# orottier/web-audio-api-rs

Measured on AMD Instinct MI355X. Metric: render quanta/sec (48kHz, 128-frame), higher is better.
Workload: dtype f64

## Files before the change

### web-audio-api-rs_amd/csrc/waa_biquad_stream.hip

```cpp
#include <hip/hip_runtime.h>

#include <cstdlib>

#include "waa_internal.hpp"
#include "waa_stream_common.hpp"

namespace waa {

namespace {
struct M2 {
  double a, b, c, d;
};
__device__ __forceinline__ M2 mm(const M2& x, const M2& y) {
  M2 r;
  r.a = __builtin_fma(x.a, y.a, x.b * y.c);
  r.b = __builtin_fma(x.a, y.b, x.b * y.d);
  r.c = __builtin_fma(x.c, y.a, x.d * y.c);
  r.d = __builtin_fma(x.c, y.b, x.d * y.d);
  return r;
}

}

__device__ unsigned long long g_stream_trace[8192 * 4];

template <int DBG, int VARY, int NBUF = 2, bool DUP = false>
__global__ __launch_bounds__(64, 2) void biquad_stream_kernel_t(const BiquadStreamDesc d) {
  extern __shared__ __attribute__((aligned(16))) float lds[];
  const uint32_t wid = blockIdx.x;
  const uint32_t inst = wid / (uint32_t)d.nch;
  const int ch = (int)(wid % (uint32_t)d.nch);
  const int lane = threadIdx.x;
  if (inst >= d.n_inst) return;

  __builtin_amdgcn_s_setreg(1 | (6 << 6) | (1 << 11), 0);
  unsigned long long trace_t0 = 0;
  if constexpr (DBG == 7) trace_t0 = wall_clock64();

  const double* cp = d.coefs + (uint64_t)inst * d.coef_stride;
  double b0 = cp[0], b1 = cp[1], b2 = cp[2], a1 = cp[3], a2 = cp[4];
  M2 A1;
  {
    M2 m = {-a1, -a2, 1., 0.};
#pragma unroll
    for (int s = 0; s < 5; s++) m = mm(m, m);
    A1 = m;
  }
  const M2 A2 = mm(A1, A1), A4 = mm(A2, A2), A8 = mm(A4, A4), A16 = mm(A8, A8);
  M2 Aj = {1., 0., 0., 1.};
  if constexpr (VARY == 0) {
    const int j = lane & 15;
    if (j & 1) Aj = mm(Aj, A1);
    if (j & 2) Aj = mm(Aj, A2);
    if (j & 4) Aj = mm(Aj, A4);
    if (j & 8) Aj = mm(Aj, A8);
  }
  const int row = lane >> 4;

  double* st = d.state + (uint64_t)inst * STATE_STRIDE + ch * 4;
  double cx1 = st[0], cx2 = st[1], cy1 = st[2], cy2 = st[3];

  float g[2] = {1.f, 1.f};
  bool g_mute[2] = {false, false}, g_pass[2] = {true, true};
#pragma unroll
  for (int k = 0; k < 2; k++)
    if (k < d.n_gain) {
      g[k] = d.gain[k].base[inst];
      g_mute[k] = fabsf(g[k]) <= 1e-6f;
      g_pass[k] = fabsf(1.f - g[k]) <= 1e-6f;
    }

  const bool is_src = d.in.kind == IN_SOURCE;
  SrcInst si{};
  SrcSchedule sc{};
  const float* sig_base = nullptr;
  if (is_src) {
    si = d.in.src[inst];
    sc = si.sc;
  } else {
    sig_base = d.in.sig.base + (uint64_t)inst * d.in.sig.inst_stride + (uint64_t)ch * d.in.sig.ch_stride;
  }
  float* out_base = d.out.base + (uint64_t)inst * d.out.inst_stride + (uint64_t)ch * d.out.ch_stride;

  auto lds_sync = []() __attribute__((always_inline)) { __builtin_amdgcn_wave_barrier(); };

  auto fetch_fast = [&](uint32_t tile, float (&dst)[TILE_K]) __attribute__((always_inline)) {
    const float* p = is_src ? si.base + (uint64_t)ch * si.ch_stride +
                                  (tile < si.fast_prefix ? si.linear_start + (int64_t)tile * TILE
                                                         : load_global(&sc.qrec[(uint64_t)tile * QUANTA_PER_TILE].start))
                            : sig_base + (uint64_t)tile * TILE;
#pragma unroll
    for (int j = 0; j < NV4; j++) {
      const f4v t = DBG == 5 ? load_global_f4(p + j * 256 + lane * 4)
                             : __builtin_nontemporal_load((const WAA_GLOBAL_AS f4v*)(p + j * 256 + lane * 4));
      dst[j * 4 + 0] = t.x;
      dst[j * 4 + 1] = t.y;
      dst[j * 4 + 2] = t.z;
      dst[j * 4 + 3] = t.w;
    }
  };
  auto tile_is_fast = [&](uint32_t tile) __attribute__((always_inline)) -> bool {
    return !is_src || tile < si.fast_prefix || (si.aligned && load_global(sc.tile_fast + tile));
  };

  auto stage = [&](const float (&cur)[TILE_K]) __attribute__((always_inline)) {
#pragma unroll
    for (int j = 0; j < NV4; j++) {
      const int r = j * 8 + (lane >> 3), c = (lane & 7) * 4;
      *reinterpret_cast<float4*>(lds + r * LDS_ROW + c) =
          make_float4(cur[j * 4 + 0], cur[j * 4 + 1], cur[j * 4 + 2], cur[j * 4 + 3]);
    }
  };
  float* lds_out = lds + 64 * LDS_ROW;
  auto flush = [&](uint32_t tile) __attribute__((always_inline)) {
    lds_sync();
    float* op = out_base + (uint64_t)tile * TILE;
#pragma unroll
    for (int j = 0; j < NV4; j++) {
      const int r = j * 8 + (lane >> 3), c = (lane & 7) * 4;
      float4 t = *reinterpret_cast<const float4*>(lds_out + r * LDS_ROW + c);
#pragma unroll
      for (int k = 0; k < 2; k++)
        if (k < d.n_gain) {
          if (g_mute[k]) {
            t = make_float4(0.f, 0.f, 0.f, 0.f);
          } else if (!g_pass[k]) {
            t.x *= g[k];
            t.y *= g[k];
            t.z *= g[k];
            t.w *= g[k];
          }
        }
      if constexpr (DBG == 2) {
        asm volatile("" ::"v"(t.x), "v"(t.y), "v"(t.z), "v"(t.w));
      } else if constexpr (DBG == 5) {
        *reinterpret_cast<float4*>(op + j * 256 + lane * 4) = t;
      } else {
        __builtin_nontemporal_store(f4v{t.x, t.y, t.z, t.w}, (WAA_GLOBAL_AS f4v*)(op + j * 256 + lane * 4));
        if constexpr (DUP)
          __builtin_nontemporal_store(f4v{t.x, t.y, t.z, t.w}, (WAA_GLOBAL_AS f4v*)(op + d.out.ch_stride + j * 256 + lane * 4));
      }
    }
    lds_sync();
  };
  auto process_arate = [&](uint32_t tile) __attribute__((always_inline)) {
    lds_sync();
    const float* xrow = lds + lane * LDS_ROW;
    float* yrow = lds_out + lane * LDS_ROW;
    const double* ct = cp + (uint64_t)tile * (TILE_K * 5 * 64) + lane;
    auto load_chunk = [&](double (&c)[20], int chunk) __attribute__((always_inline)) {
      if (DBG >= 3 && tile != d.tile0) return;
#pragma unroll
      for (int j = 0; j < 20; j++) c[j] = load_global(ct + (chunk * 20 + j) * 64);
    };
    const float xl1 = xrow[TILE_K - 1], xl2 = xrow[TILE_K - 2];
    const float xm1 = __shfl_up(xl1, 1, 64), xm2 = __shfl_up(xl2, 1, 64);
// ... 127 lines not shown
            load_chunk(ca, chunk + 3);
            step_b(cb, chunk + 1);
            load_chunk(cb, chunk + 4);
            step_b(cc, chunk + 2);
          }
          step_b(ca, 6);
          step_b(cb, 7);
        } else {
#pragma unroll 1
          for (int chunk = 0; chunk < TILE_K / 4; chunk += 2) {
            step_b(ca, chunk);
            if (chunk + 2 < TILE_K / 4) load_chunk(ca, chunk + 2);
            step_b(cb, chunk + 1);
            if (chunk + 3 < TILE_K / 4) load_chunk(cb, chunk + 3);
          }
        }
      };
      sweep(false);
      if (__any(badacc != badacc)) {
        y1 = __builtin_isfinite(s1) ? s1 : 0.;
        y2 = __builtin_isfinite(s2) ? s2 : 0.;
        load_chunk(ca, 0);
        load_chunk(cb, 1);
        sweep(true);
      }
      cx1 = (double)__int_as_float(__builtin_amdgcn_readlane(__float_as_int(xl1), 63));
      cx2 = (double)__int_as_float(__builtin_amdgcn_readlane(__float_as_int(xl2), 63));
      cy1 = read_lane(y1, 63);
      cy2 = read_lane(y2, 63);
    }
    lds_sync();
  };
  auto process = [&](uint32_t tile) __attribute__((always_inline)) {
    lds_sync();
    float x[TILE_K];
#pragma unroll
    for (int j = 0; j < NV4; j++) {
      const float4 t = *reinterpret_cast<const float4*>(lds + lane * LDS_ROW + j * 4);
      x[j * 4 + 0] = t.x;
      x[j * 4 + 1] = t.y;
      x[j * 4 + 2] = t.z;
      x[j * 4 + 3] = t.w;
    }
    if constexpr (DBG == 1) {
      lds_sync();
#pragma unroll
      for (int j = 0; j < NV4; j++)
        *reinterpret_cast<float4*>(lds_out + lane * LDS_ROW + j * 4) =
            make_float4(x[j * 4 + 0], x[j * 4 + 1], x[j * 4 + 2], x[j * 4 + 3]);
      lds_sync();
      return;
    }
    M2 Al = A1;
    if constexpr (VARY == 1) {
      uint32_t q = tile * QUANTA_PER_TILE + (lane >> 2);
      if (q >= d.n_quanta) q = d.n_quanta - 1;
      const double* cq = cp + (uint64_t)q * 5;
      b0 = cq[0];
      b1 = cq[1];
      b2 = cq[2];
      a1 = cq[3];
      a2 = cq[4];
      M2 m = {-a1, -a2, 1., 0.};
#pragma unroll
      for (int s = 0; s < 5; s++) m = mm(m, m);
      Al = m;
    }
    const float xm1 = __shfl_up(x[TILE_K - 1], 1, 64), xm2 = __shfl_up(x[TILE_K - 2], 1, 64);
    double x1 = lane == 0 ? cx1 : (double)xm1;
    double x2 = lane == 0 ? cx2 : (double)xm2;
    double w[TILE_K];
    double z1 = 0., z2 = 0.;
#pragma unroll
    for (int i = 0; i < TILE_K; i++) {
      const double xd = (double)x[i];
      w[i] = (b0 * xd + b1 * x1) + b2 * x2;
      x2 = x1;
      x1 = xd;
      const double t = __builtin_fma(-a2, z2, w[i]);
      const double y = __builtin_fma(-a1, z1, t);
      z2 = z1;
      z1 = y;
    }
    double s1, s2;
    if constexpr (VARY == 0) {
      double r1 = z1, r2 = z2;
      {
        double q1 = row_shr<1>(r1), q2 = row_shr<1>(r2);
        r1 = __builtin_fma(A1.a, q1, __builtin_fma(A1.b, q2, r1));
        r2 = __builtin_fma(A1.c, q1, __builtin_fma(A1.d, q2, r2));
        q1 = row_shr<2>(r1);
        q2 = row_shr<2>(r2);
        r1 = __builtin_fma(A2.a, q1, __builtin_fma(A2.b, q2, r1));
        r2 = __builtin_fma(A2.c, q1, __builtin_fma(A2.d, q2, r2));
        q1 = row_shr<4>(r1);
        q2 = row_shr<4>(r2);
        r1 = __builtin_fma(A4.a, q1, __builtin_fma(A4.b, q2, r1));
        r2 = __builtin_fma(A4.c, q1, __builtin_fma(A4.d, q2, r2));
        q1 = row_shr<8>(r1);
        q2 = row_shr<8>(r2);
        r1 = __builtin_fma(A8.a, q1, __builtin_fma(A8.b, q2, r1));
        r2 = __builtin_fma(A8.c, q1, __builtin_fma(A8.d, q2, r2));
      }
      const double e01 = read_lane(r1, 15), e02 = read_lane(r2, 15);
      const double e11 = read_lane(r1, 31), e12 = read_lane(r2, 31);
      const double e21 = read_lane(r1, 47), e22 = read_lane(r2, 47);
      const double t01 = cy1, t02 = cy2;
      const double t11 = __builtin_fma(A16.a, t01, __builtin_fma(A16.b, t02, e01));
      const double t12 = __builtin_fma(A16.c, t01, __builtin_fma(A16.d, t02, e02));
      const double t21 = __builtin_fma(A16.a, t11, __builtin_fma(A16.b, t12, e11));
      const double t22 = __builtin_fma(A16.c, t11, __builtin_fma(A16.d, t12, e12));
      const double t31 = __builtin_fma(A16.a, t21, __builtin_fma(A16.b, t22, e21));
      const double t32 = __builtin_fma(A16.c, t21, __builtin_fma(A16.d, t22, e22));
      const double T1 = row == 0 ? t01 : row == 1 ? t11 : row == 2 ? t21 : t31;
      const double T2 = row == 0 ? t02 : row == 1 ? t12 : row == 2 ? t22 : t32;
      const double ex1 = row_shr<1>(r1), ex2 = row_shr<1>(r2);
      s1 = __builtin_fma(Aj.a, T1, __builtin_fma(Aj.b, T2, ex1));
      s2 = __builtin_fma(Aj.c, T1, __builtin_fma(Aj.d, T2, ex2));
    } else {
      M2 P = Al;
      double r1 = z1, r2 = z2;
      auto step = [&](auto shr) __attribute__((always_inline)) {
        M2 Q;
        Q.a = shr(P.a, 1.);
        Q.b = shr(P.b, 0.);
        Q.c = shr(P.c, 0.);
        Q.d = shr(P.d, 1.);
        const double q1 = shr(r1, 0.), q2 = shr(r2, 0.);
        r1 = __builtin_fma(P.a, q1, __builtin_fma(P.b, q2, r1));
        r2 = __builtin_fma(P.c, q1, __builtin_fma(P.d, q2, r2));
        P = mm(P, Q);
      };
      step([](double v, double idv) __attribute__((always_inline)) { return row_shr_keep<1>(v, idv); });
      step([](double v, double idv) __attribute__((always_inline)) { return row_shr_keep<2>(v, idv); });
      step([](double v, double idv) __attribute__((always_inline)) { return row_shr_keep<4>(v, idv); });
      step([](double v, double idv) __attribute__((always_inline)) { return row_shr_keep<8>(v, idv); });
      double t1[4], t2[4];
      t1[0] = cy1;
      t2[0] = cy2;
#pragma unroll
      for (int k = 0; k < 3; k++) {
        const int e = 16 * k + 15;
        const double pa = read_lane(P.a, e), pb = read_lane(P.b, e), pc = read_lane(P.c, e), pd = read_lane(P.d, e);
        const double e1 = read_lane(r1, e), e2 = read_lane(r2, e);
        t1[k + 1] = __builtin_fma(pa, t1[k], __builtin_fma(pb, t2[k], e1));
        t2[k + 1] = __builtin_fma(pc, t1[k], __builtin_fma(pd, t2[k], e2));
      }
      const double T1 = row == 0 ? t1[0] : row == 1 ? t1[1] : row == 2 ? t1[2] : t1[3];
      const double T2 = row == 0 ? t2[0] : row == 1 ? t2[1] : row == 2 ? t2[2] : t2[3];
      const double xa = row_shr_keep<1>(P.a, 1.), xb = row_shr_keep<1>(P.b, 0.), xc = row_shr_keep<1>(P.c, 0.),
                   xd = row_shr_keep<1>(P.d, 1.);
      const double x1r = row_shr_keep<1>(r1, 0.), x2r = row_shr_keep<1>(r2, 0.);
      s1 = __builtin_fma(xa, T1, __builtin_fma(xb, T2, x1r));
      s2 = __builtin_fma(xc, T1, __builtin_fma(xd, T2, x2r));
    }
    double y1 = s1, y2 = s2;
    float badacc = 0.f;
    float yo[TILE_K];
#pragma unroll
    for (int i = 0; i < TILE_K; i++) {
      const double y = (w[i] - a1 * y1) - a2 * y2;
      y2 = y1;
      y1 = y;
      yo[i] = (float)y;
      badacc = __builtin_fmaf(yo[i], 0.f, badacc);
    }
    if (__any(badacc != badacc)) {
      y1 = s1;
      y2 = s2;
      if (!__builtin_isfinite(y1)) y1 = 0.;
      if (!__builtin_isfinite(y2)) y2 = 0.;
#pragma unroll
      for (int i = 0; i < TILE_K; i++) {
        double y = (w[i] - a1 * y1) - a2 * y2;
        if (!__builtin_isnormal(y)) y = 0.;
        y2 = y1;
        y1 = y;
        yo[i] = (float)y;
      }
    }
    cx1 = (double)__int_as_float(__builtin_amdgcn_readlane(__float_as_int(x[TILE_K - 1]), 63));
    cx2 = (double)__int_as_float(__builtin_amdgcn_readlane(__float_as_int(x[TILE_K - 2]), 63));
    cy1 = read_lane(y1, 63);
    cy2 = read_lane(y2, 63);
    lds_sync();
#pragma unroll
    for (int j = 0; j < NV4; j++)
      *reinterpret_cast<float4*>(lds_out + lane * LDS_ROW + j * 4) =
          make_float4(yo[j * 4 + 0], yo[j * 4 + 1], yo[j * 4 + 2], yo[j * 4 + 3]);
    lds_sync();
  };

  bool pending = false;
  uint32_t pending_tile = 0;
  uint32_t tile = d.tile0;
  while (tile < d.tile1) {
    if (!tile_is_fast(tile)) {
      float tmp[TILE_K];
      load_channel_generic(d.in, si, sc, ch, tile, lane, d.n_quanta, tmp);
      float cur[TILE_K];
#pragma unroll
      for (int i = 0; i < TILE_K; i++) cur[i] = tmp[i];
      stage(cur);
      if (pending) flush(pending_tile);
      if constexpr (VARY >= 2) process_arate(tile); else process(tile);
      pending = true;
      pending_tile = tile;
      tile++;
      continue;
    }
    uint32_t end = tile + 1;
    if (is_src && end < si.fast_prefix) end = si.fast_prefix < d.tile1 ? si.fast_prefix : d.tile1;
    while (end < d.tile1 && tile_is_fast(end)) end++;
    if constexpr (VARY == 0 && NBUF == 4) {
      float na[TILE_K], nb[TILE_K];
      fetch_fast(tile, na);
      fetch_fast(tile + 1 < end ? tile + 1 : tile, nb);
      for (; tile + 1 < end; tile += 2) {
        stage(na);
        fetch_fast(tile + 2 < end ? tile + 2 : tile, na);
        if (pending) flush(pending_tile);
        process(tile);
        pending = true;
        pending_tile = tile;
        stage(nb);
        fetch_fast(tile + 3 < end ? tile + 3 : tile + 1, nb);
        flush(pending_tile);
        process(tile + 1);
        pending_tile = tile + 1;
      }
      if (tile < end) {
        stage(na);
        if (pending) flush(pending_tile);
        process(tile);
        pending = true;
        pending_tile = tile;
        tile++;
      }
      continue;
    }
    float nx[TILE_K];
    fetch_fast(tile, nx);
    for (; tile < end; tile++) {
      stage(nx);
      fetch_fast(tile + 1 < end ? tile + 1 : tile, nx);
      if (pending) flush(pending_tile);
      if constexpr (VARY >= 2) process_arate(tile); else process(tile);
      pending = true;
      pending_tile = tile;
    }
  }
  if (pending) flush(pending_tile);
  if (lane == 0) {
    st[0] = cx1;
    st[1] = cx2;
    st[2] = cy1;
    st[3] = cy2;
  }
  if constexpr (DBG == 7) {
    if (lane == 0 && wid < 8192) {
      g_stream_trace[wid * 4 + 0] = trace_t0;
      g_stream_trace[wid * 4 + 1] = wall_clock64();
      g_stream_trace[wid * 4 + 2] = __builtin_amdgcn_s_getreg(4 | (0 << 6) | (31 << 11));
      g_stream_trace[wid * 4 + 3] = __builtin_amdgcn_s_getreg(20 | (0 << 6) | (31 << 11));
    }
  }
}

__global__ __launch_bounds__(64, 4) void biquad_stream_digest_kernel(const BiquadStreamDesc d) {
  extern __shared__ __attribute__((aligned(16))) float lds[];
  double* htab = reinterpret_cast<double*>(lds + 64 * LDS_ROW);
  const uint32_t wid = blockIdx.x;
  const uint32_t inst = wid / (uint32_t)d.nch;
  const int ch = (int)(wid % (uint32_t)d.nch);
  const int lane = threadIdx.x;
  if (inst >= d.n_inst) return;
  __builtin_amdgcn_s_setreg(1 | (6 << 6) | (1 << 11), 0);

  auto uni = [](double v) __attribute__((always_inline)) {
    return __hiloint2double(__builtin_amdgcn_readfirstlane(__double2hiint(v)), __builtin_amdgcn_readfirstlane(__double2loint(v)));
  };
  auto uni_m = [&](const M2& m) __attribute__((always_inline)) { return M2{uni(m.a), uni(m.b), uni(m.c), uni(m.d)}; };
  const double* cp = d.coefs + (uint64_t)inst * d.coef_stride;
  const double b0 = uni(cp[0]), b1 = uni(cp[1]), b2 = uni(cp[2]), a1 = uni(cp[3]), a2 = uni(cp[4]);
  M2 A1;
  {
    M2 m = {-a1, -a2, 1., 0.};
#pragma unroll
    for (int s = 0; s < 5; s++) m = mm(m, m);
    A1 = uni_m(m);
  }
  const M2 A2 = uni_m(mm(A1, A1)), A4 = uni_m(mm(A2, A2)), A8 = uni_m(mm(A4, A4)), A16 = uni_m(mm(A8, A8));
  M2 Aj = {1., 0., 0., 1.};
  {
    const int j = lane & 15;
    if (j & 1) Aj = mm(Aj, A1);
    if (j & 2) Aj = mm(Aj, A2);
    if (j & 4) Aj = mm(Aj, A4);
    if (j & 8) Aj = mm(Aj, A8);
  }
// ... 238 lines not shown
    if (!tile_is_fast(tile)) {
      float tmp[TILE_K];
      load_channel_generic(d.in, si, sc, ch, tile, lane, d.n_quanta, tmp);
      float cur[TILE_K];
#pragma unroll
      for (int i = 0; i < TILE_K; i++) cur[i] = tmp[i];
      swap_in(cur, have, done);
      process();
      have = true;
      done = tile;
      tile++;
      continue;
    }
    uint32_t end = tile + 1;
    if (is_src && end < si.fast_prefix) end = si.fast_prefix < d.tile1 ? si.fast_prefix : d.tile1;
    while (end < d.tile1 && tile_is_fast(end)) end++;
    float nx[TILE_K];
    fetch_fast(tile, nx);
    for (; tile < end; tile++) {
      swap_in(nx, have, done);
      fetch_fast(tile + 1 < end ? tile + 1 : tile, nx);
      process();
      have = true;
      done = tile;
    }
  }
  if (have) flush_last(done);
  if (lane == 0) {
    st[0] = cx1;
    st[1] = cx2;
    st[2] = cy1;
    st[3] = cy2;
  }
}

void launch_biquad_stream(const BiquadStreamDesc& d, void* stream) {
  const dim3 grid(d.n_inst * (uint32_t)d.nch), block(64);
  const size_t lds = 2 * 64 * LDS_ROW * sizeof(float);
  const char* dbg = measure_switch("WAA_STREAM_DEBUG");
  if (d.dup_out && d.vary == 0) {
    hipLaunchKernelGGL((biquad_stream_kernel_t<0, 0, 4, true>), grid, block, lds, (hipStream_t)stream, d);
    return;
  }
  if (d.vary == 3 && dbg && dbg[0] == '3')
    hipLaunchKernelGGL((biquad_stream_kernel_t<3, 3>), grid, block, lds, (hipStream_t)stream, d);
  else if (d.vary == 3 && dbg && dbg[0] == '4')
    hipLaunchKernelGGL((biquad_stream_kernel_t<4, 3>), grid, block, lds, (hipStream_t)stream, d);
  else if (d.vary == 3 && measure_switch("WAA_ARATE_BUFS3"))
    hipLaunchKernelGGL((biquad_stream_kernel_t<0, 3, 3>), grid, block, lds, (hipStream_t)stream, d);
  else if (d.vary == 3)
    hipLaunchKernelGGL((biquad_stream_kernel_t<0, 3>), grid, block, lds, (hipStream_t)stream, d);
  else if (d.vary == 2)
    hipLaunchKernelGGL((biquad_stream_kernel_t<0, 2>), grid, block, lds, (hipStream_t)stream, d);
  else if (d.vary)
    hipLaunchKernelGGL((biquad_stream_kernel_t<0, 1>), grid, block, lds, (hipStream_t)stream, d);
  else if (dbg && dbg[0] == '1')
    hipLaunchKernelGGL((biquad_stream_kernel_t<1, 0>), grid, block, lds, (hipStream_t)stream, d);
  else if (dbg && dbg[0] == '2')
    hipLaunchKernelGGL((biquad_stream_kernel_t<2, 0>), grid, block, lds, (hipStream_t)stream, d);
  else if (dbg && dbg[0] == '5')
    hipLaunchKernelGGL((biquad_stream_kernel_t<5, 0>), grid, block, lds, (hipStream_t)stream, d);
  else if (dbg && dbg[0] == '7')
    hipLaunchKernelGGL((biquad_stream_kernel_t<7, 0>), grid, block, lds, (hipStream_t)stream, d);
  else if (measure_switch("WAA_STREAM_PREFETCH1"))
    hipLaunchKernelGGL((biquad_stream_kernel_t<0, 0, 2>), grid, block, lds, (hipStream_t)stream, d);
  else if (measure_switch("WAA_BIQUAD_DIGEST"))
    hipLaunchKernelGGL(biquad_stream_digest_kernel, grid, block, 64 * LDS_ROW * sizeof(float) + 34 * 2 * sizeof(double),
                       (hipStream_t)stream, d);
  else
    hipLaunchKernelGGL((biquad_stream_kernel_t<0, 0, 4>), grid, block, lds, (hipStream_t)stream, d);
}

}

extern "C" int waa_debug_stream_trace(unsigned long long* dst, unsigned n_words) {
  return (int)hipMemcpyFromSymbol(dst, HIP_SYMBOL(waa::g_stream_trace), (size_t)n_words * 8);
}
```

### web-audio-api-rs_amd/csrc/waa_internal.hpp

```cpp
#pragma once
#include <cstdint>
#include <cstdlib>

#include "waa_conv_noise.hpp"

namespace waa {

inline const char* measure_switch(const char* name) {
#ifdef WAA_MEASURE
  return getenv(name);
#else
  (void)name;
  return nullptr;
#endif
}

void raise_lds_limit(const void* kernel);

constexpr int RQ = 128;
constexpr int TILE_K = 32;
constexpr int TILE = 64 * TILE_K;
constexpr int QUANTA_PER_TILE = TILE / RQ;
constexpr int MAX_OPS = 12;
constexpr int MAX_INPUTS = 4;
// ... 78 lines not shown
  int32_t nch_out;
  int32_t i1;
  int32_t i2;
  int32_t i0;
  ParamRef p0;
  ParamRef p1;
  ParamRef p2;
  ParamRef p3;
  ParamRef p4;
  const void* ptr0;
  void* ptr1;
  const void* ptr2;
  uint64_t u0;
};

struct ChainDesc {
  int32_t n_inputs;
  int32_t in_nch;
  int32_t in_interp;
  int32_t n_ops;
  InputRef in[MAX_INPUTS];
  OpDesc ops[MAX_OPS];
  SignalRef out;
  uint32_t n_inst;
  uint32_t n_tiles;
  uint32_t n_quanta;
  uint32_t xcd_remap;
  uint32_t tile0, tile1;
  int32_t lds_curve_op;
  int32_t tile_major;
  uint32_t persist_block;
  uint32_t pad;
};

struct BiquadStreamDesc {
  InputRef in;
  const double* coefs;
  uint64_t coef_stride;
  int32_t vary;
  int32_t pad0;
  double* state;
  const double* hp;
  ParamRef gain[2];
  int32_t n_gain;
  int32_t nch;
  SignalRef out;
  uint32_t n_inst;
  uint32_t n_tiles;
  uint32_t n_quanta;
  uint32_t dup_out;
  uint32_t tile0, tile1;
};
void launch_biquad_stream(const BiquadStreamDesc& d, void* stream);
constexpr int BIQUAD_SCAN_PW = 88;
struct BiquadScanCtl {
  uint32_t* counter;
  uint32_t counter_base[8];
  double* payload;
  const double* pw;
  uint32_t* error;
};
void launch_biquad_scan_powers(const double* coefs, uint64_t coef_stride, double* pw, uint32_t n_inst, void* stream);
void launch_biquad_scan(const BiquadStreamDesc& d, const BiquadScanCtl& ctl, uint32_t* issued, void* stream);

constexpr int BIQUAD_HT_WORDS = 2 * TILE + 8;
struct BiquadLanesDesc {
  InputRef in;
  const double* coefs;
  double* ht;
  double* z;
  double* sin;
  double* state;
  ParamRef gain[2];
  int32_t n_gain, nch;
  SignalRef out;
  uint32_t n_inst, n_tiles, n_quanta, tile0, tile1;
  uint32_t fast_tiles;
  uint32_t lt0, lt1;
  uint32_t debug, pad;
};
void launch_biquad_tile_digest(const BiquadLanesDesc& d, void* stream);
void launch_biquad_lanes(const BiquadLanesDesc& d, void* stream);

struct IirStreamDesc {
  InputRef in;
  const double* coef;
  const double* pow;
  double* state;
  int32_t ns;
  int32_t nch;
  SignalRef out;
  uint32_t n_inst;
  uint32_t n_tiles;
  uint32_t n_quanta;
  uint32_t exact;
  uint32_t tile0, tile1;
};
int iir_padded_states(int n_states);
void launch_iir_stream(const IirStreamDesc& d, void* stream);

struct CompRow {
  float thr, lo, hi, half_knee;
  float knee_partial, ratio, makeup, pad;
  float a_tau, a_one, r_tau, r_one;
};
struct CompDesc {
// ... 524 lines not shown
```

### web-audio-api-rs_amd/csrc/waa_plan.cpp

```cpp
#include <array>
#include <set>

#include <memory>

#include "waa_host.hpp"
#include "waa_plan_parts.hpp"

namespace waa {
namespace host {

int prepare_source_input(waa_batch* b, uint32_t id, InputRef* in);
int validate_plan(waa_batch* b);

int device_timeline_param(waa_batch* b, const ParamStore& p, ParamRef* ref) {
  if (p.dev_ready) {
    *ref = p.dev_ref;
    return 0;
  }
  std::vector<TlHeader> hdr(b->n_inst);
  std::vector<TlEvent> events;
  std::vector<float> curves;
  for (uint32_t i = 0; i < b->n_inst; i++) {
    TlHeader& h = hdr[i];
    std::memset(&h, 0, sizeof h);
// ... 705 lines not shown
      for (size_t k = i + 1; k < j; k++) L.gain[k - i - 1] = ops[k].p0;
      L.nch = cur_nch;
      L.out = seg_out;
      L.n_inst = b->n_inst;
      L.n_tiles = b->n_tiles;
      L.n_quanta = b->n_quanta;
      L.tile0 = 0;
      L.tile1 = b->n_tiles;
      L.fast_tiles = inputs[0].kind == IN_SOURCE ? inputs[0].fast_tiles
                                                 : (inputs[0].valid ? (uint32_t)std::min<uint64_t>(inputs[0].valid / TILE, b->n_tiles) : b->n_tiles);
      dstep.kind = 18;
      dstep.lanes = L;
      dstep.profile_slot = slot_for(b, "biquad_tile_digest_kernel");
      Step ls;
      ls.kind = 19;
      ls.lanes = L;
      ls.profile_slot = slot_for(b, "biquad_lanes_kernel");
      b->steps.push_back(ls);
      plan_note(b, "biquad_lanes(a-rate, shared table: one lane per stream, tiles in parallel) in=%s:%dch gains=%d out=%s",
                input_kind_name(inputs[0].kind), cur_nch, L.n_gain, seg_out.base == out.base ? "final" : "temp");
      InputRef in{};
      in.kind = IN_SIGNAL;
      in.nch = cur_nch;
      in.sig = seg_out;
      inputs.assign(1, in);
      in_nch = cur_nch;
      i = j;
      if (i == ops.size() && seg_out.base == out.base) return 0;
      continue;
    }
    Step st;
    st.kind = 1;
    BiquadStreamDesc& q = st.bq;
    std::memset(&q, 0, sizeof q);
    q.in = inputs[0];
    q.coefs = reinterpret_cast<const double*>(o.ptr0);
    q.coef_stride = o.u0;
    q.vary = o.i0;
    if (o.i0 == 2) {
      Step& cstep = b->steps[(size_t)o.i1];
      cstep.coef.lane_major = 1;
      if (cstep.coef.rows == 1 && !measure_switch("WAA_NO_ARATE_DIGEST")) {
        Step& hstep = b->steps[(size_t)o.i1 + 1];
        double* dhp = nullptr;
        int e = dev_alloc(b, &dhp, (size_t)b->n_tiles * HP_WORDS * 64);
        if (e) return e;
        hstep.hp.coefs = cstep.coef.coefs;
        hstep.hp.hp = dhp;
        hstep.hp.n_tiles = b->n_tiles;
        q.hp = dhp;
        q.vary = 3;
      }
    }
    q.state = reinterpret_cast<double*>(o.ptr1);
    q.n_gain = (int)(j - i - 1);
    for (size_t k = i + 1; k < j; k++) q.gain[k - i - 1] = ops[k].p0;
    q.nch = cur_nch;
    q.out = seg_out;
    q.dup_out = dup ? 1u : 0u;
    q.n_inst = b->n_inst;
    q.n_tiles = b->n_tiles;
    q.tile0 = 0;
    q.tile1 = b->n_tiles;
    q.n_quanta = b->n_quanta;
    st.profile_slot = slot_for(b, "biquad_stream_kernel");
    if (q.vary == 0 && !b->dry && measure_switch("WAA_BIQUAD_SCAN")) {
      const size_t n_streams = (size_t)b->n_inst * cur_nch;
      if (!b->scan_counter) {
        int e = dev_alloc(b, &b->scan_counter, 8 * 16 + 16);
        if (e) return e;
        b->state_bufs.push_back({b->scan_counter, (8 * 16 + 16) * sizeof(uint32_t)});
      }
      double *payload = nullptr, *pw = nullptr;
      int e;
      if ((e = dev_alloc(b, &payload, n_streams * b->n_tiles * 8)) || (e = dev_alloc(b, &pw, (size_t)b->n_inst * BIQUAD_SCAN_PW)))
        return e;
      b->ones_bufs.push_back({payload, n_streams * b->n_tiles * 8 * sizeof(double)});
      launch_biquad_scan_powers(q.coefs, q.coef_stride, pw, b->n_inst, b->stream);
      HIP_TRY(hipGetLastError());
      st.scan.counter = b->scan_counter;
      st.scan.error = b->scan_counter + 8 * 16;
      st.scan.payload = payload;
      st.scan.pw = pw;
      st.profile_slot = slot_for(b, "biquad_scan_kernel");
    }
    b->steps.push_back(st);
    if (dup) {
      plan_note(b, "biquad_stream in=%s:1ch gains=%d out=final (both channels: the speakers up-mix 1 -> 2 behind it)",
                input_kind_name(inputs[0].kind), q.n_gain);
      return 0;
    }
    plan_note(b, "biquad_stream%s in=%s:%dch gains=%d out=%s",
              q.vary == 3 ? "(a-rate, shared table)" : q.vary == 2 ? "(a-rate, per-instance table)" : q.vary ? "(k-rate)" : "",
              input_kind_name(inputs[0].kind),
              cur_nch, q.n_gain, seg_out.base == out.base ? "final" : "temp");
    InputRef in{};
    in.kind = IN_SIGNAL;
    in.nch = cur_nch;
    in.sig = seg_out;
    inputs.assign(1, in);
    in_nch = cur_nch;
    i = j;
    if (i == ops.size() && seg_out.base == out.base) return 0;
  }
  return push_chain_step(b, inputs, in_nch, in_interp, pending, out);
}

bool is_delay(const waa_batch* b, uint32_t id) { return b->nodes[id].desc.kind == WAA_NODE_DELAY; }
void vertex_targets(const waa_batch* b, uint32_t v, const std::vector<uint8_t>& cut, std::vector<uint32_t>& out) {
  const uint32_t id = v & ~VTX_READER;
  if (!(v & VTX_READER) && is_delay(b, id)) {
    if (!cut[id]) out.push_back(id | VTX_READER);
    return;
  }
  for (auto& e : b->edges) {
    if (e.from != id) continue;
    out.push_back(is_delay(b, e.to) && (e.to_input & 0x80000000u) ? (e.to | VTX_READER) : e.to);
  }
}

int materialise_automation(waa_batch* b) {
  const double sample_rate = (double)b->sr, dt = 1. / sample_rate;
  for (Node& n : b->nodes)
    for (size_t pk = 0; pk < n.params.size(); pk++) {
      ParamStore& p = n.params[pk];
      if (p.timelines.empty()) continue;
      bool shared = p.timelines_shared && p.timelines[0];
      for (uint32_t i = 1; i < b->n_inst && shared; i++) shared = p.cst[i] == p.cst[0] && p.timelines[i];
      {
        const uint32_t kind = n.desc.kind;
        const bool consumable = kind == WAA_NODE_GAIN || kind == WAA_NODE_BIQUAD || kind == WAA_NODE_DELAY ||
                                kind == WAA_NODE_STEREO_PANNER || kind == WAA_NODE_CONSTANT_SOURCE ||
                                kind == WAA_NODE_OSCILLATOR ||
                                (kind == WAA_NODE_PANNER && pk >= 6 && n.desc.i[0] != WAA_PANNING_HRTF);
        const bool want = measure_switch("WAA_DEVICE_AUTOMATION") ? true : !shared;
        bool arrivals = false;
        for (const auto& tl : p.timelines) arrivals |= tl && tl->has_arrivals();
        if (consumable && !p.k_rate && want && !arrivals && !b->dry && !measure_switch("WAA_HOST_AUTOMATION")) {
          p.dev_tl = true;
          continue;
        }
      }
      for (uint32_t inst = 0; inst < (shared ? 1u : b->n_inst); inst++) {
        Timeline* tl = p.timelines[inst].get();
        if (!tl) continue;
        float buf[RQ];
        ParamBlock run;
        run.inst = shared ? WAA_ALL_INSTANCES : inst;
// ... 1243 lines not shown
```

### web-audio-api-rs_amd/csrc/waa_plan_ops.cpp

```cpp
#include <array>
#include <set>

#include "waa_host.hpp"
#include "waa_plan_parts.hpp"

namespace waa {
namespace host {

int emit_node_ops(waa_batch* b, uint32_t id, int cur_nch, bool head, std::vector<OpDesc>& ops, int* out_nch) {
  Node& n = b->nodes[id];
  const uint32_t kind = n.desc.kind;
  if (kind == WAA_NODE_BUFFER_SOURCE || kind == WAA_NODE_CONSTANT_SOURCE) {
    *out_nch = n.out_nch;
    return 0;
  }
  if (!head && cur_nch != n.in_nch) {
    OpDesc m{};
    m.kind = OP_MIX;
    m.nch_in = cur_nch;
    m.nch_out = n.in_nch;
    m.i0 = n.interp;
    ops.push_back(m);
  }
  const int nch = n.in_nch;
// ... 15 lines not shown
      bool varies = false, a_rate = false;
      for (size_t k = 0; k < n.params.size(); k++) {
        if (param_mode(n, k) == 2) a_rate = true;
        if (param_mode(n, k) == 1) varies = true;
      }
      if (a_rate) {
        Step cs;
        cs.kind = 5;
        BiquadCoefDesc& cdsc = cs.coef;
        std::memset(&cdsc, 0, sizeof cdsc);
        int e;
        if ((e = node_param(b, id, WAA_PARAM_BIQUAD_FREQUENCY, &cdsc.frequency)) ||
            (e = node_param(b, id, WAA_PARAM_BIQUAD_DETUNE, &cdsc.detune)) ||
            (e = node_param(b, id, WAA_PARAM_BIQUAD_Q, &cdsc.q)) ||
            (e = node_param(b, id, WAA_PARAM_BIQUAD_GAIN, &cdsc.gain)))
          return e;
        cdsc.n_frames = (uint64_t)b->n_quanta * RQ;
        cdsc.frames_padded = b->lp;
        bool shared = true;
        for (size_t k = 0; k < 4; k++) {
          const bool modulated = k < n.pin_edges.size() && !n.pin_edges[k].empty();
          const ParamStore& ps = n.params[k];
          if (modulated || ps.dev_tl) shared = false;
          for (uint32_t i = 1; i < b->n_inst && shared; i++) shared = ps.cst[i] == ps.cst[0];
          for (auto& blk : ps.blocks) shared &= blk.inst == WAA_ALL_INSTANCES;
        }
        cdsc.rows = shared ? 1u : b->n_inst;
        cdsc.type = n.desc.i[0];
        cdsc.sample_rate = b->sr;
        double* dco = nullptr;
        if ((e = dev_alloc(b, &dco, (size_t)cdsc.rows * cdsc.frames_padded * 5))) return e;
        cdsc.coefs = dco;
        cs.profile_slot = slot_for(b, "biquad_coef_kernel");
        b->steps.push_back(cs);
        double* dst = nullptr;
        if ((e = dev_alloc(b, &dst, (size_t)b->n_inst * STATE_STRIDE))) return e;
        b->state_bufs.push_back({dst, (size_t)b->n_inst * STATE_STRIDE * sizeof(double)});
        o.i0 = 2;
        o.i1 = (int32_t)b->steps.size() - 1;
        {
          Step hs;
          hs.kind = 12;
          std::memset(&hs.hp, 0, sizeof hs.hp);
          hs.profile_slot = slot_for(b, "biquad_hp_kernel");
          b->steps.push_back(hs);
        }
        o.ptr0 = dco;
        o.ptr1 = dst;
        o.u0 = shared ? 0 : cdsc.frames_padded * 5;
        ops.push_back(o);
        break;
      }
      const uint64_t per = varies ? (uint64_t)b->n_quanta * 5 : 5;
      std::vector<double> co((size_t)b->n_inst * per);
      std::vector<float> pf, pd, pq, pg;
      for (uint32_t i = 0; i < b->n_inst; i++) {
        auto f = param_per_quantum(b, n.params[WAA_PARAM_BIQUAD_FREQUENCY], i, nullptr);
        auto d = param_per_quantum(b, n.params[WAA_PARAM_BIQUAD_DETUNE], i, nullptr);
        auto q = param_per_quantum(b, n.params[WAA_PARAM_BIQUAD_Q], i, nullptr);
        auto g = param_per_quantum(b, n.params[WAA_PARAM_BIQUAD_GAIN], i, nullptr);
        if (i > 0 && f == pf && d == pd && q == pq && g == pg) {
          std::copy(co.begin() + (size_t)(i - 1) * per, co.begin() + (size_t)i * per, co.begin() + (size_t)i * per);
          continue;
        }
        pf = f;
        pd = d;
        pq = q;
        pg = g;
        const uint32_t cnt = varies ? b->n_quanta : 1;
        for (uint32_t k = 0; k < cnt; k++) {
          auto at = [&](const std::vector<float>& v) { return v[v.size() == 1 ? 0 : k]; };
          Coefs c = biquad_coefs(n.desc.i[0], (double)b->sr, (double)computed_freq(at(f), at(d)), (double)at(g), (double)at(q));
          double* dst = &co[(size_t)i * per + (size_t)k * 5];
          dst[0] = c.b0;
          dst[1] = c.b1;
          dst[2] = c.b2;
          dst[3] = c.a1;
          dst[4] = c.a2;
        }
      }
      double* dco = nullptr;
      int e = dev_upload(b, &dco, co);
      if (e) return e;
      double* dst = nullptr;
      e = dev_alloc(b, &dst, (size_t)b->n_inst * STATE_STRIDE);
      if (e) return e;
      b->state_bufs.push_back({dst, (size_t)b->n_inst * STATE_STRIDE * sizeof(double)});
      o.i0 = varies ? 1 : 0;
      o.ptr0 = dco;
      o.ptr1 = dst;
      o.u0 = per;
      ops.push_back(o);
      break;
    }
    case WAA_NODE_IIR_FILTER: {
      OpDesc o{};
      o.kind = OP_IIR;
      o.nch_in = o.nch_out = nch;
      const int len = (int)n.iir_b.size();
      const int ns = iir_padded_states(len - 1);
      if (ns < 0) return fail(WAA_ERR_DEVICE, "internal: IIR order");
      std::vector<double> co(2 * (size_t)(ns + 1), 0.);
      for (int k = 0; k < len; k++) {
        co[k] = n.iir_b[k];
        co[ns + 1 + k] = n.iir_a[k];
      }
      std::vector<DD> m((size_t)ns * ns), t((size_t)ns * ns);
      for (int i = 0; i < ns; i++) {
        m[(size_t)i * ns] = DD{-co[ns + 1 + i + 1], 0.};
        if (i + 1 < ns) m[(size_t)i * ns + i + 1] = dd_add(m[(size_t)i * ns + i + 1], DD{1., 0.});
      }
      double growth = 0.;
      auto note = [&](const std::vector<DD>& a) {
        for (const DD& v : a) growth = std::isfinite(v.hi) ? std::max(growth, std::fabs(v.hi)) : INFINITY;
      };
      auto mul = [&](const std::vector<DD>& x, const std::vector<DD>& y, std::vector<DD>& out) {
        for (int r = 0; r < ns; r++)
          for (int c = 0; c < ns; c++) {
            DD acc{0., 0.};
            for (int k = 0; k < ns; k++) acc = dd_add(acc, dd_mul(x[(size_t)r * ns + k], y[(size_t)k * ns + c]));
            out[(size_t)r * ns + c] = acc;
          }
      };
      for (int k = 0; k < 5; k++) {
        mul(m, m, t);
        m.swap(t);
        note(m);
      }
      const std::vector<DD> A = m;
      std::vector<double> pw(6 * (size_t)ns * ns);
      for (int lvl = 0; lvl < 6; lvl++) {
        for (size_t k = 0; k < (size_t)ns * ns; k++) pw[lvl * (size_t)ns * ns + k] = m[k].hi + m[k].lo;
        mul(m, m, t);
        m.swap(t);
        note(m);
      }
      m = A;
      for (int j = 2; j <= 64 && std::isfinite(growth); j++) {
        mul(m, A, t);
        m.swap(t);
        note(m);
      }
      const char* genv = measure_switch("WAA_IIR_GROWTH");
      const double growth_limit = genv ? atof(genv) : 1e4;
// ... 208 lines not shown
```

Measured before the change: 2.952 billion.

## Precompute k-rate biquad scan matrices in a plan-time table kernel

For k-rate biquads whose coefficients are identical across instances, the host now uploads a single shared coefficient row instead of one per instance. A separate table kernel is launched once at plan time and precomputes, per tile, the coefficients, the power-of-two scan matrices and the segment end matrices. The stream kernel gains a VARY==4 path that loads these from the table, prefetching the next tile's coefficients, instead of recomputing the matrix powers and products every tile. This trades repeated double-precision matrix work per tile for extra global loads and a one-time table build, and it changes the flush/fetch ordering for this path.

```diff
diff --git a/web-audio-api-rs_amd/csrc/waa_biquad_stream.hip b/web-audio-api-rs_amd/csrc/waa_biquad_stream.hip
--- a/web-audio-api-rs_amd/csrc/waa_biquad_stream.hip
+++ b/web-audio-api-rs_amd/csrc/waa_biquad_stream.hip
@@ -22,10 +22,65 @@
 
 }
 
+__global__ __launch_bounds__(64) void biquad_krate_table_kernel(const double* coefs, double* tab, uint32_t n_quanta) {
+  const uint32_t tile = blockIdx.x;
+  const int lane = threadIdx.x;
+  __builtin_amdgcn_s_setreg(1 | (6 << 6) | (1 << 11), 0);
+  uint32_t q = tile * QUANTA_PER_TILE + (lane >> 2);
+  if (q >= n_quanta) q = n_quanta - 1;
+  const double* cq = coefs + (uint64_t)q * 5;
+  const double b0 = cq[0], b1 = cq[1], b2 = cq[2], a1 = cq[3], a2 = cq[4];
+  double* t = tab + (uint64_t)tile * BIQUAD_KT_WORDS + lane;
+  t[0 * 64] = b0;
+  t[1 * 64] = b1;
+  t[2 * 64] = b2;
+  t[3 * 64] = a1;
+  t[4 * 64] = a2;
+  M2 P = {-a1, -a2, 1., 0.};
+#pragma unroll
+  for (int s = 0; s < 5; s++) P = mm(P, P);
+  int word = 5;
+  auto put = [&](const M2& m) __attribute__((always_inline)) {
+    t[(word + 0) * 64] = m.a;
+    t[(word + 1) * 64] = m.b;
+    t[(word + 2) * 64] = m.c;
+    t[(word + 3) * 64] = m.d;
+    word += 4;
+  };
+  auto step = [&](auto shr) __attribute__((always_inline)) {
+    put(P);
+    M2 Q;
+    Q.a = shr(P.a, 1.);
+    Q.b = shr(P.b, 0.);
+    Q.c = shr(P.c, 0.);
+    Q.d = shr(P.d, 1.);
+    P = mm(P, Q);
+  };
+  step([](double v, double idv) __attribute__((always_inline)) { return row_shr_keep<1>(v, idv); });
+  step([](double v, double idv) __attribute__((always_inline)) { return row_shr_keep<2>(v, idv); });
+  step([](double v, double idv) __attribute__((always_inline)) { return row_shr_keep<4>(v, idv); });
+  step([](double v, double idv) __attribute__((always_inline)) { return row_shr_keep<8>(v, idv); });
+  M2 X;
+  X.a = row_shr_keep<1>(P.a, 1.);
+  X.b = row_shr_keep<1>(P.b, 0.);
+  X.c = row_shr_keep<1>(P.c, 0.);
+  X.d = row_shr_keep<1>(P.d, 1.);
+  put(X);
+  double* ends = tab + (uint64_t)tile * BIQUAD_KT_WORDS + 25 * 64;
+  if ((lane & 15) == 15) {
+    const int k = lane >> 4;
+    ends[k * 4 + 0] = P.a;
+    ends[k * 4 + 1] = P.b;
+    ends[k * 4 + 2] = P.c;
+    ends[k * 4 + 3] = P.d;
+  }
+}
+
 __device__ unsigned long long g_stream_trace[8192 * 4];
 
 template <int DBG, int VARY, int NBUF = 2, bool DUP = false>
 __global__ __launch_bounds__(64, 2) void biquad_stream_kernel_t(const BiquadStreamDesc d) {
+  constexpr bool KTAB = VARY == 4, ARATE = VARY == 2 || VARY == 3;
   extern __shared__ __attribute__((aligned(16))) float lds[];
   const uint32_t wid = blockIdx.x;
   const uint32_t inst = wid / (uint32_t)d.nch;
@@ -102,6 +157,24 @@
   auto tile_is_fast = [&](uint32_t tile) __attribute__((always_inline)) -> bool {
     return !is_src || tile < si.fast_prefix || (si.aligned && load_global(sc.tile_fast + tile));
   };
+
+  double kt[20], kcur[5], knext[5], kte = 0., kte_next = 0.;
+  auto ktab_request_next = [&](uint32_t tile) __attribute__((always_inline)) {
+    const double* np = d.hp + (uint64_t)(tile < d.n_tiles ? tile : d.n_tiles - 1) * BIQUAD_KT_WORDS;
+#pragma unroll
+    for (int k = 0; k < 5; k++) knext[k] = load_global(np + k * 64 + lane);
+    kte_next = load_global(np + 25 * 64 + (lane & 15));
+  };
+  auto ktab_fetch = [&](uint32_t tile) __attribute__((always_inline)) {
+    const double* tp = d.hp + (uint64_t)tile * BIQUAD_KT_WORDS;
+#pragma unroll
+    for (int k = 0; k < 5; k++) kcur[k] = knext[k];
+    kte = kte_next;
+#pragma unroll
+    for (int k = 0; k < 20; k++) kt[k] = load_global(tp + (5 + k) * 64 + lane);
+    ktab_request_next(tile + 1);
+  };
+  if constexpr (KTAB) ktab_request_next(d.tile0);
 
   auto stage = [&](const float (&cur)[TILE_K]) __attribute__((always_inline)) {
 #pragma unroll
@@ -335,7 +408,13 @@
       return;
     }
     M2 Al = A1;
-    if constexpr (VARY == 1) {
+    if constexpr (KTAB) {
+      b0 = kcur[0];
+      b1 = kcur[1];
+      b2 = kcur[2];
+      a1 = kcur[3];
+      a2 = kcur[4];
+    } else if constexpr (VARY == 1) {
       uint32_t q = tile * QUANTA_PER_TILE + (lane >> 2);
       if (q >= d.n_quanta) q = d.n_quanta - 1;
       const double* cq = cp + (uint64_t)q * 5;
@@ -400,6 +479,42 @@
       const double ex1 = row_shr<1>(r1), ex2 = row_shr<1>(r2);
       s1 = __builtin_fma(Aj.a, T1, __builtin_fma(Aj.b, T2, ex1));
       s2 = __builtin_fma(Aj.c, T1, __builtin_fma(Aj.d, T2, ex2));
+    } else if constexpr (KTAB) {
+      double r1 = z1, r2 = z2;
+      {
+        double q1 = row_shr_keep<1>(r1, 0.), q2 = row_shr_keep<1>(r2, 0.);
+        r1 = __builtin_fma(kt[0], q1, __builtin_fma(kt[1], q2, r1));
+        r2 = __builtin_fma(kt[2], q1, __builtin_fma(kt[3], q2, r2));
+        q1 = row_shr_keep<2>(r1, 0.);
+        q2 = row_shr_keep<2>(r2, 0.);
+        r1 = __builtin_fma(kt[4], q1, __builtin_fma(kt[5], q2, r1));
+        r2 = __builtin_fma(kt[6], q1, __builtin_fma(kt[7], q2, r2));
+        q1 = row_shr_keep<4>(r1, 0.);
+        q2 = row_shr_keep<4>(r2, 0.);
+        r1 = __builtin_fma(kt[8], q1, __builtin_fma(kt[9], q2, r1));
+        r2 = __builtin_fma(kt[10], q1, __builtin_fma(kt[11], q2, r2));
+        q1 = row_shr_keep<8>(r1, 0.);
+        q2 = row_shr_keep<8>(r2, 0.);
+        r1 = __builtin_fma(kt[12], q1, __builtin_fma(kt[13], q2, r1));
+        r2 = __builtin_fma(kt[14], q1, __builtin_fma(kt[15], q2, r2));
+      }
+      double t1[4], t2[4];
+      t1[0] = cy1;
+      t2[0] = cy2;
+#pragma unroll
+      for (int k = 0; k < 3; k++) {
+        const int e = 16 * k + 15;
+        const double pa = read_lane(kte, 4 * k), pb = read_lane(kte, 4 * k + 1), pc = read_lane(kte, 4 * k + 2),
+                     pd = read_lane(kte, 4 * k + 3);
+        const double e1 = read_lane(r1, e), e2 = read_lane(r2, e);
+        t1[k + 1] = __builtin_fma(pa, t1[k], __builtin_fma(pb, t2[k], e1));
+        t2[k + 1] = __builtin_fma(pc, t1[k], __builtin_fma(pd, t2[k], e2));
+      }
+      const double T1 = row == 0 ? t1[0] : row == 1 ? t1[1] : row == 2 ? t1[2] : t1[3];
+      const double T2 = row == 0 ? t2[0] : row == 1 ? t2[1] : row == 2 ? t2[2] : t2[3];
+      const double x1r = row_shr_keep<1>(r1, 0.), x2r = row_shr_keep<1>(r2, 0.);
+      s1 = __builtin_fma(kt[16], T1, __builtin_fma(kt[17], T2, x1r));
+      s2 = __builtin_fma(kt[18], T1, __builtin_fma(kt[19], T2, x2r));
     } else {
       M2 P = Al;
       double r1 = z1, r2 = z2;
@@ -477,6 +592,17 @@
   bool pending = false;
   uint32_t pending_tile = 0;
   uint32_t tile = d.tile0;
+  auto before_fetch = [&](uint32_t t) __attribute__((always_inline)) {
+    if constexpr (KTAB) {
+      if (pending) flush(pending_tile);
+      ktab_fetch(t);
+    }
+  };
+  auto after_fetch = [&]() __attribute__((always_inline)) {
+    if constexpr (!KTAB) {
+      if (pending) flush(pending_tile);
+    }
+  };
   while (tile < d.tile1) {
     if (!tile_is_fast(tile)) {
       float tmp[TILE_K];
@@ -485,8 +611,9 @@
 #pragma unroll
       for (int i = 0; i < TILE_K; i++) cur[i] = tmp[i];
       stage(cur);
-      if (pending) flush(pending_tile);
-      if constexpr (VARY >= 2) process_arate(tile); else process(tile);
+      before_fetch(tile);
+      after_fetch();
+      if constexpr (ARATE) process_arate(tile); else process(tile);
       pending = true;
       pending_tile = tile;
       tile++;
@@ -495,26 +622,29 @@
     uint32_t end = tile + 1;
     if (is_src && end < si.fast_prefix) end = si.fast_prefix < d.tile1 ? si.fast_prefix : d.tile1;
     while (end < d.tile1 && tile_is_fast(end)) end++;
-    if constexpr (VARY == 0 && NBUF == 4) {
+    if constexpr ((VARY == 0 || KTAB) && NBUF == 4) {
       float na[TILE_K], nb[TILE_K];
       fetch_fast(tile, na);
       fetch_fast(tile + 1 < end ? tile + 1 : tile, nb);
       for (; tile + 1 < end; tile += 2) {
         stage(na);
+        before_fetch(tile);
         fetch_fast(tile + 2 < end ? tile + 2 : tile, na);
-        if (pending) flush(pending_tile);
+        after_fetch();
         process(tile);
         pending = true;
         pending_tile = tile;
         stage(nb);
+        before_fetch(tile + 1);
         fetch_fast(tile + 3 < end ? tile + 3 : tile + 1, nb);
-        flush(pending_tile);
+        after_fetch();
         process(tile + 1);
         pending_tile = tile + 1;
       }
       if (tile < end) {
         stage(na);
-        if (pending) flush(pending_tile);
+        before_fetch(tile);
+        after_fetch();
         process(tile);
         pending = true;
         pending_tile = tile;
@@ -526,9 +656,10 @@
     fetch_fast(tile, nx);
     for (; tile < end; tile++) {
       stage(nx);
+      before_fetch(tile);
       fetch_fast(tile + 1 < end ? tile + 1 : tile, nx);
-      if (pending) flush(pending_tile);
-      if constexpr (VARY >= 2) process_arate(tile); else process(tile);
+      after_fetch();
+      if constexpr (ARATE) process_arate(tile); else process(tile);
       pending = true;
       pending_tile = tile;
     }
@@ -873,6 +1004,10 @@
     hipLaunchKernelGGL((biquad_stream_kernel_t<0, 3>), grid, block, lds, (hipStream_t)stream, d);
   else if (d.vary == 2)
     hipLaunchKernelGGL((biquad_stream_kernel_t<0, 2>), grid, block, lds, (hipStream_t)stream, d);
+  else if (d.vary && d.hp && measure_switch("WAA_KRATE_PREFETCH1"))
+    hipLaunchKernelGGL((biquad_stream_kernel_t<0, 4, 2>), grid, block, lds, (hipStream_t)stream, d);
+  else if (d.vary && d.hp)
+    hipLaunchKernelGGL((biquad_stream_kernel_t<0, 4, 4>), grid, block, lds, (hipStream_t)stream, d);
   else if (d.vary)
     hipLaunchKernelGGL((biquad_stream_kernel_t<0, 1>), grid, block, lds, (hipStream_t)stream, d);
   else if (dbg && dbg[0] == '1')
@@ -892,6 +1027,11 @@
     hipLaunchKernelGGL((biquad_stream_kernel_t<0, 0, 4>), grid, block, lds, (hipStream_t)stream, d);
 }
 
+
+void launch_biquad_krate_table(const double* coefs, double* tab, uint32_t n_tiles, uint32_t n_quanta, void* stream) {
+  hipLaunchKernelGGL(biquad_krate_table_kernel, dim3(n_tiles), dim3(64), 0, (hipStream_t)stream, coefs, tab, n_quanta);
+}
+
 }
 
 extern "C" int waa_debug_stream_trace(unsigned long long* dst, unsigned n_words) {
diff --git a/web-audio-api-rs_amd/csrc/waa_internal.hpp b/web-audio-api-rs_amd/csrc/waa_internal.hpp
--- a/web-audio-api-rs_amd/csrc/waa_internal.hpp
+++ b/web-audio-api-rs_amd/csrc/waa_internal.hpp
@@ -154,6 +154,8 @@
   uint32_t tile0, tile1;
 };
 void launch_biquad_stream(const BiquadStreamDesc& d, void* stream);
+constexpr int BIQUAD_KT_WORDS = 25 * 64 + 16;
+void launch_biquad_krate_table(const double* coefs, double* tab, uint32_t n_tiles, uint32_t n_quanta, void* stream);
 constexpr int BIQUAD_SCAN_PW = 88;
 struct BiquadScanCtl {
   uint32_t* counter;
diff --git a/web-audio-api-rs_amd/csrc/waa_plan.cpp b/web-audio-api-rs_amd/csrc/waa_plan.cpp
--- a/web-audio-api-rs_amd/csrc/waa_plan.cpp
+++ b/web-audio-api-rs_amd/csrc/waa_plan.cpp
@@ -781,6 +781,16 @@
         q.vary = 3;
       }
     }
+    if (o.i0 == 1 && o.u0 == 0 && !measure_switch("WAA_KRATE_INLINE")) {
+      double* kt = nullptr;
+      int e = dev_alloc(b, &kt, (size_t)b->n_tiles * BIQUAD_KT_WORDS);
+      if (e) return e;
+      if (!b->dry) {
+        launch_biquad_krate_table(q.coefs, kt, b->n_tiles, b->n_quanta, b->stream);
+        HIP_TRY(hipGetLastError());
+      }
+      q.hp = kt;
+    }
     q.state = reinterpret_cast<double*>(o.ptr1);
     q.n_gain = (int)(j - i - 1);
     for (size_t k = i + 1; k < j; k++) q.gain[k - i - 1] = ops[k].p0;
@@ -823,6 +833,10 @@
               q.vary == 3 ? "(a-rate, shared table)" : q.vary == 2 ? "(a-rate, per-instance table)" : q.vary ? "(k-rate)" : "",
               input_kind_name(inputs[0].kind),
               cur_nch, q.n_gain, seg_out.base == out.base ? "final" : "temp");
+    if (q.vary == 1)
+      plan_note(b, "k-rate coefficients: %s", q.hp               ? "one row for the batch, scan matrices from the plan-time table"
+                                              : q.coef_stride == 0 ? "one row for the batch, scan matrices in the kernel"
+                                                                   : "a row per instance, scan matrices in the kernel");
     InputRef in{};
     in.kind = IN_SIGNAL;
     in.nch = cur_nch;
diff --git a/web-audio-api-rs_amd/csrc/waa_plan_ops.cpp b/web-audio-api-rs_amd/csrc/waa_plan_ops.cpp
--- a/web-audio-api-rs_amd/csrc/waa_plan_ops.cpp
+++ b/web-audio-api-rs_amd/csrc/waa_plan_ops.cpp
@@ -91,7 +91,8 @@
         break;
       }
       const uint64_t per = varies ? (uint64_t)b->n_quanta * 5 : 5;
-      std::vector<double> co((size_t)b->n_inst * per);
+      bool shared = varies;
+      std::vector<double> co((size_t)(shared ? 1 : b->n_inst) * per);
       std::vector<float> pf, pd, pq, pg;
       for (uint32_t i = 0; i < b->n_inst; i++) {
         auto f = param_per_quantum(b, n.params[WAA_PARAM_BIQUAD_FREQUENCY], i, nullptr);
@@ -99,8 +100,13 @@
         auto q = param_per_quantum(b, n.params[WAA_PARAM_BIQUAD_Q], i, nullptr);
         auto g = param_per_quantum(b, n.params[WAA_PARAM_BIQUAD_GAIN], i, nullptr);
         if (i > 0 && f == pf && d == pd && q == pq && g == pg) {
-          std::copy(co.begin() + (size_t)(i - 1) * per, co.begin() + (size_t)i * per, co.begin() + (size_t)i * per);
+          if (!shared) std::copy(co.begin() + (size_t)(i - 1) * per, co.begin() + (size_t)i * per, co.begin() + (size_t)i * per);
           continue;
+        }
+        if (shared && i > 0) {
+          shared = false;
+          co.resize((size_t)b->n_inst * per);
+          for (uint32_t r = 1; r < i; r++) std::copy(co.begin(), co.begin() + per, co.begin() + (size_t)r * per);
         }
         pf = f;
         pd = d;
@@ -128,7 +134,7 @@
       o.i0 = varies ? 1 : 0;
       o.ptr0 = dco;
       o.ptr1 = dst;
-      o.u0 = per;
+      o.u0 = shared ? 0 : per;
       ops.push_back(o);
       break;
     }
```

Result: slower. 2.915 billion (-1.3%).
